# probcomp/PClean

Measured on AMD Instinct MI355X. Metric: rows/sec per Gibbs sweep on 1M-row synthetic hospital; F1 vs ground truth, higher is better.
Workload: dtype f64

## Files before the change

pclean_amd/csrc/sweep.hip:

```cpp
#include "sweep_internal.h"

int g_pclean_sync_count = 0;

__global__ void publish_count_kernel(const unsigned int* __restrict__ src, volatile unsigned int* __restrict__ dst, unsigned int seq) {
  dst[0] = *src;
  __threadfence_system();
  dst[1] = seq;
}
int read_count(pclean_ctx* ctx, const void* dev, void* out, const char* func, int line) {
  SweepState* s = st(ctx);
  static const bool no_poll = getenv("PCLEAN_NO_POLL") != nullptr;
  static const bool trace = getenv("PCLEAN_TRACE_SYNC") != nullptr;
  if (trace) fprintf(stderr, "[pclean sync %d] %s:%d (count)\n", ++g_pclean_sync_count, func, line);
  if (!no_poll && !s->h_poll) {
    if (hipHostMalloc((void**)&s->h_poll, 64, hipHostMallocMapped | hipHostMallocCoherent) != hipSuccess) s->h_poll = nullptr;
    if (s->h_poll) {
      s->h_poll[0] = s->h_poll[1] = 0;
      if (hipHostGetDevicePointer((void**)&s->d_poll, (void*)s->h_poll, 0) != hipSuccess) {
        (void)hipHostFree((void*)s->h_poll);
        s->h_poll = nullptr;
      }
    }
  }
  if (no_poll || !s->h_poll) {
    HIPCHK(ctx, hipMemcpyAsync(out, dev, 4, hipMemcpyDeviceToHost, ctx->stream));
    HIPCHK(ctx, hipStreamSynchronize(ctx->stream));
    return PCLEAN_OK;
  }
  const unsigned int seq = ++s->poll_seq;
  hipLaunchKernelGGL(publish_count_kernel, dim3(1), dim3(1), 0, ctx->stream, (const unsigned int*)dev, s->d_poll, seq);
  if (s->on_first_wait) {
    std::function<int()> f;
    f.swap(s->on_first_wait);
    const int rcf = f();
    if (rcf) return rcf;
  }
  volatile unsigned int* h = s->h_poll;
  for (long spins = 0; h[1] != seq; ++spins)
    if (spins > 2000000) {
      HIPCHK(ctx, hipStreamSynchronize(ctx->stream));
      if (h[1] != seq) return pclean_fail(ctx, PCLEAN_ERR_HIP, "count read-back: the publishing kernel did not run");
    }
  *(unsigned int*)out = h[0];
  return PCLEAN_OK;
}

__device__ int32_t resolve_new_value(const PlanDev& pl, int node, int col, const int32_t* vals) {
  for (int depth = 0; depth < 16; ++depth) {
    const int cn = pl.colmap[2 * (pl.colmap_begin[node] + col)];
    const int cc = pl.colmap[2 * (pl.colmap_begin[node] + col) + 1];
    if (cn < 0) return -1;
    const int choice = vals[cn];
    if (pl.kind[cn] == PCLEAN_NODE_LEAF) return pl.cols[cn][choice];
    if (choice >= 0) return pl.cols[cn][(size_t)cc * pl.n_rows[cn] + choice];
    node = cn;
    col = cc;
  }
  return -1;
}




struct CtxSrc {
  int32_t n_ctx;
  const int32_t* pchoice[PCLEAN_MAX_CTX];
  const int32_t* pnewpos[PCLEAN_MAX_CTX];
  const int32_t* vals[PCLEAN_MAX_CTX];
  int32_t n_nodes[PCLEAN_MAX_CTX];
  const int32_t* root_col[PCLEAN_MAX_CTX];
  int32_t col[PCLEAN_MAX_CTX];
  PlanDev plan[PCLEAN_MAX_CTX];
};

__global__ void gather_ctx_kernel(size_t NP, CtxSrc cs, int32_t* it_ctx) {
  size_t t = (size_t)blockIdx.x * blockDim.x + threadIdx.x;
  if (t >= NP) return;
  for (int s = 0; s < cs.n_ctx; ++s) {
    int32_t v;
    const int choice = cs.pchoice[s][t];
    if (choice >= 0)
      v = cs.root_col[s][choice];
    else
      v = resolve_new_value(cs.plan[s], 0, cs.col[s], cs.vals[s] + (size_t)cs.pnewpos[s][t] * cs.n_nodes[s]);
    it_ctx[(size_t)s * NP + t] = v;
  }
}

__global__ void ctx_count_kernel(int N, int P, int n_ctx, const int32_t* __restrict__ it_ctx, int32_t* __restrict__ rep,
                                 int32_t* __restrict__ n_distinct) {
  const int i = blockIdx.x * blockDim.x + threadIdx.x;
  if (i >= N) return;
  const size_t NP = (size_t)N * P;
  int nd = 0;
  for (int p = 0; p < P; ++p) {
    const size_t sp = (size_t)p * N + i;
    int c[PCLEAN_MAX_CTX];
    for (int k = 0; k < PCLEAN_MAX_CTX; ++k) c[k] = k < n_ctx ? it_ctx[(size_t)k * NP + sp] : 0;
    int q = 0;
    for (; q < p; ++q) {
      bool same = true;
      for (int k = 0; k < PCLEAN_MAX_CTX; ++k)
        if (k < n_ctx) same &= it_ctx[(size_t)k * NP + (size_t)q * N + i] == c[k];
      if (same) break;
    }
    rep[sp] = q;
    nd += q == p ? 1 : 0;
  }
  n_distinct[i] = nd;
}
__global__ void ctx_fill_kernel(int N, int P, int n_ctx, const int32_t* __restrict__ it_ctx, const int32_t* __restrict__ rep,
                                const int32_t* __restrict__ off, const int32_t* __restrict__ cur_b,
                                int32_t* __restrict__ slot_item, int32_t* __restrict__ row, int32_t* __restrict__ ctxv,
                                int32_t* __restrict__ excl) {
  const int i = blockIdx.x * blockDim.x + threadIdx.x;
  if (i >= N) return;
  const size_t NP = (size_t)N * P;
  int j = off[i];
  for (int p = 0; p < P; ++p) {
    const size_t sp = (size_t)p * N + i;
    const int q = rep[sp];
    if (q == p) {
      row[j] = i;
      excl[j] = cur_b ? cur_b[i] : -1;
      for (int k = 0; k < PCLEAN_MAX_CTX; ++k) ctxv[(size_t)j * PCLEAN_MAX_CTX + k] = k < n_ctx ? it_ctx[(size_t)k * NP + sp] : 0;
      slot_item[sp] = j++;
    } else {
      slot_item[sp] = slot_item[(size_t)q * N + i];
    }
  }
}
#define CI_PC 8
__global__ __launch_bounds__(256) void ctx_items_kernel(int N, int P, CtxSrc cs, const int32_t* __restrict__ cur_b,
                                                        int32_t* __restrict__ it_ctx, int32_t* __restrict__ slot_item,
                                                        int32_t* __restrict__ row, int32_t* __restrict__ ctxv,
                                                        int32_t* __restrict__ excl, unsigned int* __restrict__ n_extra,
                                                        int extra_cap) {
  __shared__ unsigned int wcnt[4];
  __shared__ unsigned int bbase;
  const int i = blockIdx.x * blockDim.x + threadIdx.x;
  const int lane = threadIdx.x & 63, wave = threadIdx.x >> 6;
  const size_t NP = (size_t)N * P;
  int c0[PCLEAN_MAX_CTX] = {0, 0, 0, 0};
  static_assert(PCLEAN_MAX_CTX == 4, "c0 initialiser");
  unsigned int mine = 0;
  if (i < N) {
    bool all_same = true;
    for (int p0 = 0; p0 < P; p0 += CI_PC) {
#pragma unroll
      for (int s = 0; s < PCLEAN_MAX_CTX; ++s) {
        if (s >= cs.n_ctx) break;
        int ch[CI_PC];
        int32_t v[CI_PC];
// ... 341 lines not shown
  if (i >= n_rows) return;
  if (only_rows && !only_rows[i]) return;
  FixW<PMAX> f;
  fix_weights<PMAX>(logw + (size_t)i * sr, sp, P, f);
  const uint32_t rr = (uint32_t)((int64_t)i + row_offset);
  const bool csmc = csmc_flag ? (csmc_flag[i] >= 0) : (is_csmc != 0);
  int c;
  if (use_mh && csmc && P >= 2) {
    const double Ud = (double)f.U;
    const double w0 = (double)f.u[0] / Ud, w1 = (double)f.u[PMAX > 1 ? 1 : 0] / Ud;
    double ratio = w1 / (1e-10 + w0);
    if (ratio > 1.0) ratio = 1.0;
    const double x = pclean_u01(pclean_rand64(seed, rr, PCLEAN_SITE_MH, 0u, sweep));
    c = (f.U != 0 && x < ratio) ? 1 : 0;
  } else {
    c = fix_pick<PMAX>(f, P, pclean_rand64(seed, rr, PCLEAN_SITE_FINAL, 0u, sweep));
  }
  chosen[i] = c;
  const double lt = pclean_lse_from_fix(f.m, f.U);
  if (log_total) log_total[i] = lt;
  if (logml) logml[i] = (logml_acc ? logml_acc[i] : 0.0) + lt - pclean_log((double)P);
}


template <int PMAX>
__global__ __launch_bounds__(256) void particle_update_final_kernel(
    int N, int P, const int32_t* __restrict__ draws_rm, const double* __restrict__ lse, const int32_t* __restrict__ slot_item,
    const int32_t* __restrict__ draws_item, const double* __restrict__ lse_item, const int32_t* __restrict__ cur_b,
    int32_t* __restrict__ pchoice, const double* __restrict__ w, int first, int use_mh, const int32_t* __restrict__ csmc_flag,
    uint64_t seed, uint32_t sweep, int64_t row_offset, int32_t* __restrict__ chosen, const double* __restrict__ logml_acc,
    double* __restrict__ logml, const int32_t* __restrict__ skip_rows, int lazy, const double* __restrict__ w_uni) {
  const int i = blockIdx.x * blockDim.x + threadIdx.x;
  if (i >= N) return;
  if (skip_rows && skip_rows[i]) return;
  const int keep = cur_b ? cur_b[i] : -1;
  if (lazy && keep >= 0) pchoice[i] = keep;
  FixW<PMAX> f;
  double wv[PMAX];
  f.m = -__builtin_inf();
  int dv[PMAX];
  double lv[PMAX], wp[PMAX];
  const size_t Ns = (size_t)N;
  if (slot_item) {
    int itm[PMAX];
#pragma unroll
    for (int p = 0; p < PMAX; ++p) itm[p] = slot_item[(size_t)(p < P ? p : P - 1) * Ns + i];
#pragma unroll
    for (int p = 0; p < PMAX; ++p) lv[p] = lse_item[itm[p]];
    if (!lazy) {
#pragma unroll
      for (int p = 0; p < PMAX; ++p) dv[p] = draws_item[(size_t)itm[p] * P + (p < P ? p : P - 1)];
    }
  } else {
    const double l0 = lse[i];
#pragma unroll
    for (int p = 0; p < PMAX; ++p) lv[p] = l0;
    if (!lazy) {
#pragma unroll
      for (int p = 0; p < PMAX; ++p) dv[p] = draws_rm[(size_t)i * P + (p < P ? p : P - 1)];
    }
  }
  if (lazy) {
#pragma unroll
    for (int p = 0; p < PMAX; ++p) dv[p] = 0;
  }
  if (first) {
#pragma unroll
    for (int p = 0; p < PMAX; ++p) wp[p] = 0.0;
  } else if (w_uni) {
    const double wu = 0.0 + w_uni[i];
#pragma unroll
    for (int p = 0; p < PMAX; ++p) wp[p] = wu;
  } else {
#pragma unroll
    for (int p = 0; p < PMAX; ++p) wp[p] = w[(size_t)(p < P ? p : P - 1) * Ns + i];
  }
#pragma unroll
  for (int p = 0; p < PMAX; ++p) {
    wv[p] = 0.0;
    if (p < P) {
      if (!lazy) pchoice[(size_t)p * Ns + i] = (p == 0 && keep >= 0) ? keep : dv[p];
      wv[p] = wp[p] + lv[p];
      f.m = fmax(f.m, wv[p]);
    }
  }
  f.U = 0;
#pragma unroll
  for (int p = 0; p < PMAX; ++p) {
    f.u[p] = (p < P && f.m != -__builtin_inf()) ? pclean_fixw(wv[p] - f.m) : 0ull;
    f.U += f.u[p];
  }
  const uint32_t rr = (uint32_t)((int64_t)i + row_offset);
  const bool csmc = csmc_flag[i] >= 0;
  int c;
  if (use_mh && csmc && P >= 2) {
    const double Ud = (double)f.U;
    const double w0 = (double)f.u[0] / Ud, w1 = (double)f.u[PMAX > 1 ? 1 : 0] / Ud;
    double ratio = w1 / (1e-10 + w0);
    if (ratio > 1.0) ratio = 1.0;
    const double x = pclean_u01(pclean_rand64(seed, rr, PCLEAN_SITE_MH, 0u, sweep));
    c = (f.U != 0 && x < ratio) ? 1 : 0;
  } else {
    c = fix_pick<PMAX>(f, P, pclean_rand64(seed, rr, PCLEAN_SITE_FINAL, 0u, sweep));
  }
  chosen[i] = c;
  logml[i] = logml_acc[i] + pclean_lse_from_fix(f.m, f.U) - pclean_log((double)P);
}

__global__ __launch_bounds__(256) void finalize_block_kernel(int n_rows, const int32_t* chosen, const int32_t* pchoice,
                                                             const int32_t* pnewpos, const int32_t* cur_b,
                                                             int32_t* choice, int32_t* chosen_newpos,
                                                             unsigned long long* stats, int hist_rows,
                                                             int32_t* moved_flag, int32_t* new_flag,
                                                             unsigned int* __restrict__ wg_moved,
                                                             unsigned int* __restrict__ wg_new) {
  extern __shared__ int32_t hist[];
  for (int k = threadIdx.x; k < hist_rows; k += 256) hist[k] = 0;
  if (hist_rows) __syncthreads();
  int i = blockIdx.x * blockDim.x + threadIdx.x;
  int is_moved = 0, is_new = 0;
  if (i < n_rows) {
    const size_t s = (size_t)chosen[i] * n_rows + i;
    const int c = pchoice[s];
    const int o = cur_b[i];
    choice[i] = c;
    const int np = c == PCLEAN_CHOICE_NEW ? pnewpos[s] : -1;
    chosen_newpos[i] = np;
    new_flag[i] = is_new = np >= 0 ? 1 : 0;
    moved_flag[i] = is_moved = c != o ? 1 : 0;
    if (o != c) {
      if (hist_rows) {
        if (o >= 0) atomicAdd(&hist[o], -1);
        if (c >= 0) atomicAdd(&hist[c], 1);
      } else {
        if (o >= 0) atomicAdd(&stats[o], (unsigned long long)(-1ll));
        if (c >= 0) atomicAdd(&stats[c], 1ull);
      }
    }
  }
  if (hist_rows) {
    __syncthreads();
    for (int k = threadIdx.x; k < hist_rows; k += 256) {
      const int v = hist[k];
      if (v) atomicAdd(&stats[k], (unsigned long long)(long long)v);
    }
  }
  const int n_moved = __syncthreads_count(is_moved), n_newr = __syncthreads_count(is_new);
  if (threadIdx.x == 0) {
    wg_moved[blockIdx.x] = (unsigned int)n_moved;
    wg_new[blockIdx.x] = (unsigned int)n_newr;
  }
}

#define TAIL_MAX_LISTS (2 * PCLEAN_MAX_BLOCKS)
__global__ __launch_bounds__(1024) void tail_scan_kernel(int nb, unsigned int* __restrict__ wg_cnt, int32_t* __restrict__ totals) {
  __shared__ unsigned int wsum[16];
  unsigned int* c = wg_cnt + (size_t)blockIdx.x * nb;
  const int lane = threadIdx.x & 63, wave = threadIdx.x >> 6;
  unsigned int carry = 0;
  for (int base = 0; base < nb; base += 1024) {
    const int j = base + threadIdx.x;
    const unsigned int v = j < nb ? c[j] : 0u;
    unsigned int incl = v;
    for (int o = 1; o < 64; o <<= 1) {
      const unsigned int x = __shfl_up(incl, o, 64);
      if (lane >= o) incl += x;
    }
    if (lane == 63) wsum[wave] = incl;
    __syncthreads();
    unsigned int wbase = 0, tot = 0;
    for (int k = 0; k < 16; ++k) {
      if (k < wave) wbase += wsum[k];
      tot += wsum[k];
    }
    if (j < nb) c[j] = carry + wbase + incl - v;
    carry += tot;
    __syncthreads();
  }
  if (threadIdx.x == 0) totals[blockIdx.x] = (int32_t)carry;
}
struct TailLists {
  const int32_t* flag[TAIL_MAX_LISTS];
  int32_t* list[TAIL_MAX_LISTS];
};
__global__ __launch_bounds__(256) void tail_scatter_kernel(int n_rows, int nb, TailLists tl, const unsigned int* __restrict__ wg_off) {
  __shared__ unsigned int wcnt[4];
  const int l = blockIdx.y;
  const int32_t* flag = tl.flag[l];
  if (!flag) return;
  const int i = blockIdx.x * 256 + threadIdx.x;
  const int lane = threadIdx.x & 63, wave = threadIdx.x >> 6;
  const bool f = i < n_rows && flag[i] != 0;
  const unsigned long long mk = __ballot(f);
  if (lane == 0) wcnt[wave] = (unsigned int)__popcll(mk);
  __syncthreads();
  if (!f) return;
  unsigned int pos = wg_off[(size_t)l * nb + blockIdx.x] + (unsigned int)__popcll(mk & ((1ull << lane) - 1ull));
  for (int w = 0; w < wave; ++w) pos += wcnt[w];
  tl.list[l][pos] = i;
}

__global__ void gauss_prior_kernel(int n_rows, int P, GaussDev g0, const GaussDev* __restrict__ more, int n_more, PlanDev plan,
                                   const int32_t* __restrict__ pchoice,
                                   const int32_t* __restrict__ pnewpos, const int32_t* __restrict__ vals, int n_nodes,
                                   const int32_t* __restrict__ cur_b, const int32_t* __restrict__ cur_locals, uint64_t seed,
                                   uint32_t sweep, uint32_t block, int64_t row_offset, double* __restrict__ w,
                                   int32_t* __restrict__ plocals) {
  const size_t slot = (size_t)blockIdx.x * blockDim.x + threadIdx.x;
  if (slot >= (size_t)n_rows * P) return;
  const int p = (int)(slot / (size_t)n_rows), i = (int)(slot % (size_t)n_rows);
  const int choice = pchoice[slot];
  const int32_t* v = choice >= 0 ? nullptr : vals + (size_t)pnewpos[slot] * n_nodes;
  const bool keep = p == 0 && cur_b && cur_b[i] >= 0 && cur_locals;
  const uint32_t rr = (uint32_t)((int64_t)i + row_offset);
  int l[2] = {0, 0}, out[2] = {-1, -1};
  double s = 0.0;
  for (int k = 0; k < g0.n_locals; ++k) {
    const int o = g0.local_obs[k] ? g0.local_obs[k][i] : -1;
    if (o >= 0) {
      l[k] = o;
      s += g0.local_logp[k];
    } else if (keep && cur_locals[2 * (size_t)i + k] >= 0) {
      l[k] = cur_locals[2 * (size_t)i + k];
    } else {
      l[k] = (int)pclean_mulhi64(pclean_rand64(seed, rr, PCLEAN_SITE_LOCALS(block), (uint32_t)p | ((uint32_t)(k + 1) << 16), sweep),
                                 (uint64_t)g0.local_n[k]);
    }
    out[k] = l[k];
  }
  plocals[2 * slot] = out[0];
  plocals[2 * slot + 1] = out[1];
  for (int t = 0; t <= n_more; ++t) {
    const GaussDev& g = t == 0 ? g0 : more[t - 1];
    const double xv = g.x[i];
    if (xv == xv) {
      int idx = 0;
      for (int d = 0; d < g.n_dims; ++d) {
        int val;
        if (g.src_kind[d] == PCLEAN_GSRC_LOCAL)
          val = l[g.src_slot[d]];
        else if (g.src_kind[d] == PCLEAN_GSRC_CAND)
          val = choice >= 0 ? g.src_ptr[d][choice] : resolve_new_value(plan, 0, g.src_slot[d], v);
        else
          val = g.src_ptr[d][i];
        idx += g.stride[d] * val;
      }
      const int u = g.t_kind == PCLEAN_GSRC_LOCAL ? l[g.t_src] : 0;
      s += gauss_normal_logpdf(g.tx[u] ? g.tx[u][i] : xv * g.t_scale[u], g.mu[idx], g.sigma, g.log_sigma);
      s -= g.tl[u] ? g.tl[u][i] : g.t_lad[u];
    }
  }
  w[slot] += s;
}
__global__ void locals_pick_kernel(int n_rows, const int32_t* __restrict__ chosen, const int32_t* __restrict__ plocals,
                                   int32_t* __restrict__ locals) {
  const int i = blockIdx.x * blockDim.x + threadIdx.x;
  if (i >= n_rows) return;
  const size_t slot = (size_t)chosen[i] * n_rows + i;
  locals[2 * i] = plocals[2 * slot];
  locals[2 * i + 1] = plocals[2 * slot + 1];
}

__global__ void locals_tail_kernel(int n_rows, int P, GaussDev g, const GaussDev* __restrict__ more, int n_more, PlanDev plan,
                                   const int32_t* chosen,
                                   const int32_t* pchoice, const int32_t* pnewpos, const int32_t* vals, int n_nodes,
                                   uint64_t seed, uint32_t sweep, uint32_t block, int64_t row_offset, int32_t* locals) {
  int i = blockIdx.x * blockDim.x + threadIdx.x;
  if (i >= n_rows) return;
  const int c = chosen[i];
  const size_t slot = (size_t)c * n_rows + i;
  const int choice = pchoice[slot];
  const int32_t* v = choice >= 0 ? nullptr : vals + (size_t)pnewpos[slot] * n_nodes;
  locals[2 * i] = locals[2 * i + 1] = -1;
  double sc[16];
  int codes[16];
  int n = gauss_combo_scores(
      g, more, n_more, i, nullptr,
      [&](const GaussDev& gt, int d) -> int {
        if (gt.src_kind[d] == PCLEAN_GSRC_CAND)
          return choice >= 0 ? gt.src_ptr[d][choice] : resolve_new_value(plan, 0, gt.src_slot[d], v);
        return gt.src_ptr[d][i];
      },
      sc, codes);
  if (n == 0) {
    for (int l0 = 0; l0 < g.local_n[0]; ++l0)
      for (int l1 = 0; l1 < g.local_n[1]; ++l1) {
        const bool ok0 = !g.local_obs[0] || g.local_obs[0][i] < 0 || g.local_obs[0][i] == l0;
        const bool ok1 = !g.local_obs[1] || g.local_obs[1][i] < 0 || g.local_obs[1][i] == l1;
        if (ok0 && ok1) {
          sc[n] = 0.0;
          codes[n] = l0 * 16 + l1;
          ++n;
        }
      }
  }
  double m = -__builtin_inf();
  for (int k = 0; k < n; ++k) m = fmax(m, sc[k]);
  uint64_t u[16], U = 0;
  for (int k = 0; k < n; ++k) {
    u[k] = m == -__builtin_inf() ? 0ull : pclean_fixw(sc[k] - m);
    U += u[k];
  }
  int pick = n - 1;
  if (U) {
    const uint64_t x = pclean_mulhi64(
        pclean_rand64(seed, (uint32_t)((int64_t)i + row_offset), PCLEAN_SITE_LOCALS(block), (uint32_t)c, sweep), U);
    uint64_t acc = 0;
// ... 1131 lines not shown
      if (!rep || !n_distinct || !off || !tmp) return pclean_fail(ctx, PCLEAN_ERR_HIP, "scratch alloc failed");
      {
        ProfScope ps(ctx, "ctx_items");
        hipLaunchKernelGGL(gather_ctx_kernel, grid1(NP), dim3(256), 0, ctx->stream, NP, cs, r.it_ctx.p);
        HIPCHK(ctx, hipMemsetAsync(n_distinct + N, 0, sizeof(int32_t), ctx->stream));
        hipLaunchKernelGGL(ctx_count_kernel, grid1(N), dim3(256), 0, ctx->stream, N, P, (int)b.n_ctx, r.it_ctx.p, rep, n_distinct);
        HIPCHK(ctx, hipcub::DeviceScan::ExclusiveSum(tmp, tmp_scan, n_distinct, off, N + 1, ctx->stream));
        PCLEAN_READ_COUNT(ctx, off + N, &n_items);
      }
      d_row = scratch<int32_t>(ctx, n_items);
      d_ctx = scratch<int32_t>(ctx, (size_t)n_items * PCLEAN_MAX_CTX);
      d_excl = scratch<int32_t>(ctx, n_items);
      if (!d_row || !d_ctx || !d_excl) return pclean_fail(ctx, PCLEAN_ERR_HIP, "scratch alloc failed");
      hipLaunchKernelGGL(ctx_fill_kernel, grid1(N), dim3(256), 0, ctx->stream, N, P, (int)b.n_ctx, r.it_ctx.p, rep, off, cur_b, slot_item,
                         d_row, d_ctx, d_excl);
      }
      double* lse_item = scratch<double>(ctx, n_items);
      int32_t* draws_item = scratch<int32_t>(ctx, (size_t)n_items * P);
      if (!lse_item || !draws_item) return pclean_fail(ctx, PCLEAN_ERR_HIP, "scratch alloc failed");
      il = ItemList{(int)n_items, d_row, d_ctx, nullptr, nullptr};
      if (!no_fused_items) il.n_primary = N;
      if (fuse_final || split_final) s->lazy_req = SweepState::LazyReq{true, split_final ? emit_rows : nullptr};
      rc = eval_node(ctx, bi, 0, il, d_excl, seed, sweep_idx, P, lse_item, draws_item, nullptr, nullptr, bi == ctx->timed_block);
      s->lazy_req = SweepState::LazyReq();
      if (rc) return rc;
      if (bi == ctx->timed_block) {
        hot_timed = true;
        ctx->timing.hot_kernel_launches += 1;
      }
      lazy = s->lazy_out;
      s->lazy_out.valid = false;
      lazy.args.slot_item = slot_item;
      ProfScope ps(ctx, "particle_update");
      if (fuse_final) {
        DISPATCH_PMAX(P, hipLaunchKernelGGL(particle_update_final_kernel<PMAX>, grid1(N), dim3(256), 0, ctx->stream, N, P,
                                            (const int32_t*)nullptr, (const double*)nullptr, slot_item, draws_item, lse_item, cur_b,
                                            r.pchoice.p, s->w.p, (w_by_first_block && bi == 0) ? 1 : 0, use_mh, cur_base, seed,
                                            sweep_idx, s->row_offset + ctx->active_begin, s->chosen.p, s->logml_acc.p, s->logml.p,
                                            (const int32_t*)nullptr, lazy.valid ? 1 : 0, w_uni));
        final_fused = true;
        { const int rcl = lazy_draws(); if (rcl) return rcl; }
      } else {
      n_new_ctr = fresh_counter(ctx);
      if (!n_new_ctr) return pclean_fail(ctx, PCLEAN_ERR_HIP, "counter bank: device alloc failed");
      hipLaunchKernelGGL(particle_update_kernel, dim3((N + PU_T - 1) / PU_T), dim3(PU_T), 0, ctx->stream, N, P, (const int32_t*)nullptr,
                         (const double*)nullptr, slot_item, draws_item, lse_item, cur_b, r.pchoice.p, s->w.p,
                         n_new_ctr, r.new_slots.p, r.pnewpos.p, (w_by_first_block && bi == 0) ? 1 : 0, emit_rows, split_final ? 1 : 0, 0,
                         w_uni, 0);
      if (!split_final) w_uni = nullptr;
      if (split_final) {
        DISPATCH_PMAX(P, hipLaunchKernelGGL(particle_update_final_kernel<PMAX>, grid1(N), dim3(256), 0, ctx->stream, N, P,
                                            (const int32_t*)nullptr, (const double*)nullptr, slot_item, draws_item, lse_item, cur_b,
                                            r.pchoice.p, s->w.p, (w_by_first_block && bi == 0) ? 1 : 0, use_mh, cur_base, seed,
                                            sweep_idx, s->row_offset + ctx->active_begin, s->chosen.p, s->logml_acc.p, s->logml.p,
                                            emit_rows, lazy.valid ? 1 : 0, w_uni));
        final_only_rows = emit_rows;
        { const int rcl = lazy_draws(); if (rcl) return rcl; }
      }
      }
    }
    if (!prefetch_started) {
      const int rcp = start_prefetch();
      if (rcp) return rcp;
    }
    unsigned int n_new = 0;
    if (!final_fused) PCLEAN_READ_COUNT(ctx, n_new_ctr, &n_new);
    const bool degenerate_rows = (n_new & 0x80000000u) != 0u;
    n_new &= 0x7fffffffu;
    r.n_new = final_fused ? -1 : (int)n_new;
    r.lazy_new = final_fused || (bi == n_blocks - 1 && !eager_all && (!drawable || emit_rows != nullptr));
    if (r.lazy_new && !emit_rows) n_new = 0;
    if (emit_rows) r.n_new = -1;
    if (r.vals.alloc(std::max<size_t>((size_t)n_new * nn, 1))) return pclean_fail(ctx, PCLEAN_ERR_HIP, "device alloc failed");
    if (n_new) {
      ProfScope ps(ctx, "new_row_sampling");
      const int32_t* list = r.new_slots.p;
      hipLaunchKernelGGL(fill_i32_kernel, grid1((size_t)n_new * nn), dim3(256), 0, ctx->stream, r.vals.p,
                         (size_t)n_new * nn, -2);
      int32_t* row = scratch<int32_t>(ctx, n_new);
      int32_t* cx = scratch<int32_t>(ctx, (size_t)n_new * PCLEAN_MAX_CTX);
      int32_t* part = scratch<int32_t>(ctx, n_new);
      int32_t* org = scratch<int32_t>(ctx, n_new);
      int32_t* ex = scratch<int32_t>(ctx, n_new);
      if (!row || !cx || !part || !org || !ex) return pclean_fail(ctx, PCLEAN_ERR_HIP, "scratch alloc failed");
      hipLaunchKernelGGL(rootlist_items_kernel, grid1(n_new), dim3(256), 0, ctx->stream, (int)n_new, N, NP, list,
                         has_ctx ? r.it_ctx.p : nullptr, cur_b, row, cx, part, org, ex);
      hipLaunchKernelGGL(set_col_kernel, grid1(n_new), dim3(256), 0, ctx->stream, (int)n_new, nn, 0,
                         (int32_t)PCLEAN_CHOICE_NEW, r.vals.p);
      ItemList sub{(int)n_new, row, cx, part, org};
      rc = sample_children(ctx, bi, 0, sub, ex, seed, sweep_idx, r.vals.p, nn);
      if (rc) return rc;
      if (prior_mode) {
        ctx->prior_mode = false;
        const NodeDev* nds;
        const int32_t *dnc, *dcb, *dch;
        rc = upload_plan_nodes(ctx, bi, &nds, &dnc, &dcb, &dch);
        if (!rc)
          rc = pclean_launch_prior_terms(ctx, NP, N, nn, nds, dnc, dcb, dch, r.pchoice.p, r.pnewpos.p, r.vals.p,
                                         has_ctx ? r.it_ctx.p : nullptr, s->w.p);
        if (!rc) rc = gauss_prior();
        if (rc) return rc;
      }
      if (drawable) {
        if (!split_final) materialise_w();
        rc = apply_dummy_corrections(ctx, bi, r.new_slots.p, r.vals.p, (int)n_new, N, seed, sweep_idx, s->w.p);
        if (rc) return rc;
      }
    } else if (prior_mode) {
      ctx->prior_mode = false;
      const NodeDev* nds;
      const int32_t *dnc, *dcb, *dch;
      rc = upload_plan_nodes(ctx, bi, &nds, &dnc, &dcb, &dch);
      if (!rc)
        rc = pclean_launch_prior_terms(ctx, NP, N, nn, nds, dnc, dcb, dch, r.pchoice.p, r.pnewpos.p, r.vals.p,
                                       has_ctx ? r.it_ctx.p : nullptr, s->w.p);
      if (!rc) rc = gauss_prior();
      if (rc) return rc;
    }
    ctx->prior_mode = false;

    const int grp_here = b.group >= 0 ? b.group : bi;
    const int grp_next = bi + 1 < n_blocks ? (ctx->block[bi + 1].group >= 0 ? ctx->block[bi + 1].group : bi + 1) : -2;
    const bool equal_weights = bi == 0 && w_by_first_block && !has_ctx && !prior_mode && !(drawable && n_new > 0) && !degenerate_rows;
    static const bool always_resample = getenv("PCLEAN_ALWAYS_RESAMPLE") != nullptr;
    if (!use_mh && bi < n_blocks - 1 && grp_here != grp_next && (!equal_weights || always_resample)) {
      ProfScope ps(ctx, "resample");
      materialise_w();
      DISPATCH_PMAX(P, hipLaunchKernelGGL(maybe_resample_kernel<PMAX>, grid1(N), dim3(256), 0, ctx->stream, N, P, s->w.p,
                                          (size_t)1, (size_t)N, 1, cur_b, seed, sweep_idx, (uint32_t)bi,
                                          s->row_offset + ctx->active_begin, s->ancestors.p, s->logml_inc.p,
                                          (double*)nullptr, s->did.p));
      AncestorArrays arrs{};
      int n_arr = 0;
      for (int k = 0; k <= bi; ++k) {
        if (ctx->block[k].is_score) continue;
        arrs.p[n_arr++] = s->run[k].pchoice.p;
        arrs.p[n_arr++] = s->run[k].pnewpos.p;
        if (s->run[k].plocals_on) arrs.pairs[arrs.n_pairs++] = reinterpret_cast<int64_t*>(s->run[k].plocals.p);
      }
      hipLaunchKernelGGL(apply_ancestors_kernel, grid1(N), dim3(256), 0, ctx->stream, N, P, s->ancestors.p, n_arr, arrs, s->w.p,
                         s->did.p, s->logml_inc.p, s->logml_acc.p);
    }
  }

  if (prefetching) HIPCHK(ctx, hipStreamWaitEvent(ctx->stream, s->pre_join, 0));
  {
    ProfScope ps(ctx, "final_choice_and_outputs");
    if (!final_fused && !final_only_rows) materialise_w();
    if (!final_fused)
    DISPATCH_PMAX(P, hipLaunchKernelGGL(final_choice_kernel<PMAX>, grid1(N), dim3(256), 0, ctx->stream, N, P, s->w.p,
                                        (size_t)1, (size_t)N, use_mh, 1, cur_base, seed, sweep_idx,
                                        s->row_offset + ctx->active_begin, s->chosen.p, (double*)nullptr,
                                        s->logml_acc.p, s->logml.p, final_only_rows));
    for (int bi = 0; bi < n_blocks; ++bi) {
      BlockRun& r = s->run[bi];
      Block& bb = ctx->block[bi];
      if (bb.is_score || !r.lazy_new || r.n_new == 0) continue;
      ProfScope ps2(ctx, "new_row_sampling_chosen");
      const int nn = (int)bb.nodes.size();
      const int32_t* cur_b = cur_base + (size_t)bi * cur_ld;
      unsigned int* cnt_ctr = fresh_counter(ctx);
      hipLaunchKernelGGL(chosen_new_kernel, grid1(N), dim3(256), 0, ctx->stream, N, s->chosen.p, r.pchoice.p, cnt_ctr,
                         r.new_slots.p, r.pnewpos.p);
      unsigned int cnt = 0;
      PCLEAN_READ_COUNT(ctx, cnt_ctr, &cnt);
      if (r.vals.alloc(std::max<size_t>((size_t)cnt * nn, 1))) return pclean_fail(ctx, PCLEAN_ERR_HIP, "device alloc failed");
      if (!cnt) continue;
      hipLaunchKernelGGL(fill_i32_kernel, grid1((size_t)cnt * nn), dim3(256), 0, ctx->stream, r.vals.p, (size_t)cnt * nn, -2);
      int32_t* row = scratch<int32_t>(ctx, cnt);
      int32_t* cx = scratch<int32_t>(ctx, (size_t)cnt * PCLEAN_MAX_CTX);
      int32_t* part = scratch<int32_t>(ctx, cnt);
      int32_t* org = scratch<int32_t>(ctx, cnt);
      int32_t* ex = scratch<int32_t>(ctx, cnt);
      if (!row || !cx || !part || !org || !ex) return pclean_fail(ctx, PCLEAN_ERR_HIP, "scratch alloc failed");
      hipLaunchKernelGGL(rootlist_items_kernel, grid1(cnt), dim3(256), 0, ctx->stream, (int)cnt, N, NP, r.new_slots.p,
                         bb.n_ctx > 0 ? r.it_ctx.p : nullptr, cur_b, row, cx, part, org, ex);
      hipLaunchKernelGGL(set_col_kernel, grid1(cnt), dim3(256), 0, ctx->stream, (int)cnt, nn, 0, (int32_t)PCLEAN_CHOICE_NEW,
                         r.vals.p);
      ItemList sub{(int)cnt, row, cx, part, org};
      int rc = sample_children(ctx, bi, 0, sub, ex, seed, sweep_idx, r.vals.p, nn);
      if (rc) return rc;
    }
    const int nb_wg = (N + 255) / 256;
    unsigned int* wg_cnt = scratch<unsigned int>(ctx, (size_t)2 * n_blocks * nb_wg);
    if (!wg_cnt) return pclean_fail(ctx, PCLEAN_ERR_HIP, "scratch alloc failed");
    TailLists tl{};
    {
      ZeroList zl{};
      for (int bi = 0; bi < n_blocks; ++bi) {
        if (ctx->block[bi].is_score) continue;
        CandTable& rt = ctx->cand[ctx->block[bi].nodes[0].table];
        bool seen = false;
        for (int k = 0; k < zl.n; ++k) seen |= zl.p[k] == (void*)rt.stats.p;
        if (!seen) zero_list_add(ctx, zl, rt.stats.p, (size_t)std::max(rt.n_rows, 1) * 8);
      }
      const int rcz = zero_list_flush(ctx, zl);
      if (rcz) return rcz;
    }
    for (int bi = 0; bi < n_blocks; ++bi) {
      BlockRun& r = s->run[bi];
      Block& bb = ctx->block[bi];
      bb.locals_host.clear();
      r.locals_rows = 0;
      if (bb.is_score) continue;
      const int32_t* cur_b = cur_base + (size_t)bi * cur_ld;
      CandTable& rt = ctx->cand[bb.nodes[0].table];
      const int rows_in_use = (rt.n_used > 0 && rt.n_used <= rt.n_rows) ? std::min(rt.n_rows, (rt.n_used + 63) & ~63) : rt.n_rows;
      static const bool no_hist = getenv("PCLEAN_NO_HIST") != nullptr;
      const int hist_rows = (rt.n_rows <= 12288 && !no_hist) ? rows_in_use : 0;
      hipLaunchKernelGGL(finalize_block_kernel, grid1(N), dim3(256), (size_t)hist_rows * sizeof(int32_t), ctx->stream, N,
                         s->chosen.p, r.pchoice.p, r.pnewpos.p, cur_b, r.choice.p, r.chosen_newpos.p,
                         (unsigned long long*)rt.stats.p, hist_rows, r.moved_flag.p, r.new_flag.p,
                         wg_cnt + (size_t)(2 * bi) * nb_wg, wg_cnt + (size_t)(2 * bi + 1) * nb_wg);
      tl.flag[2 * bi] = r.moved_flag.p;
      tl.list[2 * bi] = r.moved_list.p;
      tl.flag[2 * bi + 1] = r.new_flag.p;
      tl.list[2 * bi + 1] = r.new_list.p;
      if (choice)
        HIPCHK(ctx, hipMemcpyAsync(choice + (size_t)bi * N, r.choice.p, (size_t)N * 4, hipMemcpyDeviceToHost, ctx->stream));
      if (!bb.node_gauss.empty() && bb.node_gauss[0] >= 0 && bb.gauss[bb.node_gauss[0]].n_locals > 0) {
        if (r.locals.alloc((size_t)N * 2)) return pclean_fail(ctx, PCLEAN_ERR_HIP, "device alloc failed");
        if (r.plocals_on) {
          hipLaunchKernelGGL(locals_pick_kernel, grid1(N), dim3(256), 0, ctx->stream, N, s->chosen.p, r.plocals.p, r.locals.p);
        } else {
          GaussDev gd;
          const GaussDev* gmore;
          int n_gmore;
          int rc = build_gauss_dev(ctx, bb.gauss[bb.node_gauss[0]], &rt, gd);
          if (!rc) rc = build_gauss_more(ctx, bb, 0, &rt, &gmore, &n_gmore);
          if (rc) return rc;
          hipLaunchKernelGGL(locals_tail_kernel, grid1(N), dim3(256), 0, ctx->stream, N, P, gd, gmore, n_gmore, r.plan, s->chosen.p,
                             r.pchoice.p, r.pnewpos.p, r.vals.p, (int)bb.nodes.size(), seed, sweep_idx, (uint32_t)bi,
                             s->row_offset + ctx->active_begin, r.locals.p);
        }
        r.locals_rows = N;
        if (!defer) {
          bb.locals_host.resize((size_t)N * 2);
          HIPCHK(ctx, hipMemcpyAsync(bb.locals_host.data(), r.locals.p, (size_t)N * 8, hipMemcpyDeviceToHost, ctx->stream));
        }
      }
    }
    {
      for (int bi = 0; bi < n_blocks; ++bi)
        if (ctx->block[bi].is_score)
          HIPCHK(ctx, hipMemsetAsync(wg_cnt + (size_t)(2 * bi) * nb_wg, 0, (size_t)2 * nb_wg * sizeof(unsigned int), ctx->stream));
      hipLaunchKernelGGL(tail_scan_kernel, dim3(2 * n_blocks), dim3(1024), 0, ctx->stream, nb_wg, wg_cnt, s->tail_counts.p);
      hipLaunchKernelGGL(tail_scatter_kernel, dim3(nb_wg, 2 * n_blocks), dim3(256), 0, ctx->stream, N, nb_wg, tl, wg_cnt);
    }
    (void)hipEventRecord(s->eve, ctx->stream);
    if (chosen_particle) HIPCHK(ctx, hipMemcpyAsync(chosen_particle, s->chosen.p, (size_t)N * 4, hipMemcpyDeviceToHost, ctx->stream));
    if (logml) HIPCHK(ctx, hipMemcpyAsync(logml, s->logml.p, (size_t)N * 8, hipMemcpyDeviceToHost, ctx->stream));
  }
  s->last_hot_timed = hot_timed;
  s->outputs_pending = true;
  s->lists_on_host = false;
  {
    const Block& b0 = ctx->block[(ctx->timed_block >= 0 && ctx->timed_block < n_blocks && !ctx->block[ctx->timed_block].is_score) ? ctx->timed_block : 0];
    const double F = b0.nodes[0].n_terms, K = ctx->cand[b0.nodes[0].table].n_rows;
    ctx->timing.hot_kernel_alg_bytes = (double)N * (4.0 * F + (K + 1.0) * (8.0 * F + 4.0) + 8.0 * P);
  }
  if (defer) return PCLEAN_OK;
  int rcf = pclean_sweep_finish_queue(ctx);
  if (rcf) return rcf;
  PCLEAN_SYNC(ctx);
  rcf = pclean_sweep_finish_synced(ctx);
  if (rcf) return rcf;
  if (choice)
    for (int bi = 0; bi < n_blocks; ++bi)
      if (ctx->block[bi].is_score)
        for (int i = 0; i < N; ++i) choice[(size_t)bi * N + i] = 0;
  return pclean_sweep_fetch_lists(ctx);
}

int pclean_sweep_finish_queue(pclean_ctx* ctx) {
  SweepState* s = st(ctx);
  if (!s->outputs_pending) return PCLEAN_OK;
  int rc = d2h_small(ctx, s->h_counts, s->tail_counts.p, 2 * s->last_blocks * sizeof(int32_t));
  if (rc) return rc;
  const int rco = queue_over_copy(ctx);
  if (rco) return rco;
  s->h_counts[3 * PCLEAN_MAX_BLOCKS] = 0;
  if (s->dummy_used) rc = d2h_small(ctx, s->h_counts + 3 * PCLEAN_MAX_BLOCKS, s->dummy_ctr.p + 1, sizeof(int32_t), s->h_counts);
  if (rc) return rc;
  return d2h_flush(ctx);
}
int pclean_sweep_finish_synced(pclean_ctx* ctx) {
  SweepState* s = st(ctx);
  if (!s->outputs_pending) return PCLEAN_OK;
  s->outputs_pending = false;
  apply_over_stats(ctx);
  if (s->prof_on) prof_collect(ctx);
  float tot = 0;
  HIPCHK(ctx, hipEventElapsedTime(&tot, s->evs, s->eve));
  ctx->timing.total_ms = tot;
  ctx->timing.hot_kernel_ms = 0.f;
  if (s->last_hot_timed) {
    float ms = 0;
    HIPCHK(ctx, hipEventElapsedTime(&ms, s->ev0, s->ev1));
    ctx->timing.hot_kernel_ms = ms;
    if (s->gate_timed) {
      float mg = 0;
      HIPCHK(ctx, hipEventElapsedTime(&mg, s->evg0, s->evg1));
      ctx->timing.hot_kernel_ms += mg;
    }
  }
  if (s->h_counts[3 * PCLEAN_MAX_BLOCKS])
    return pclean_fail(ctx, PCLEAN_ERR_CAPACITY, "pclean_sweep: an observed string longer than %d symbols below a chosen "
                                                 "dummy value", DUMMY_MAX_LEN);
  return PCLEAN_OK;
}
int pclean_sweep_fetch_lists(pclean_ctx* ctx) {
  SweepState* s = st(ctx);
  if (s->lists_on_host) return PCLEAN_OK;
  for (int bi = 0; bi < s->last_blocks; ++bi) {
    BlockRun& r = s->run[bi];
    Block& b = ctx->block[bi];
    const int nn = (int)b.nodes.size();
    b.new_rows_host.clear();
    b.new_vals_host.clear();
    b.moved_rows_host.clear();
    b.moved_choice_host.clear();
    if (b.is_score) continue;
    const int n_moved = s->h_counts[2 * bi], n_newrows = s->h_counts[2 * bi + 1];
    if (n_moved > 0) {
      int32_t* ch_d = scratch<int32_t>(ctx, n_moved);
      if (!ch_d) return pclean_fail(ctx, PCLEAN_ERR_HIP, "scratch alloc failed");
      hipLaunchKernelGGL(gather_moved_kernel, grid1(n_moved), dim3(256), 0, ctx->stream, n_moved, r.moved_list.p,
                         r.choice.p, ch_d);
      b.moved_rows_host.resize(n_moved);
      b.moved_choice_host.resize(n_moved);
      HIPCHK(ctx, hipMemcpyAsync(b.moved_rows_host.data(), r.moved_list.p, (size_t)n_moved * 4, hipMemcpyDeviceToHost, ctx->stream));
      HIPCHK(ctx, hipMemcpyAsync(b.moved_choice_host.data(), ch_d, (size_t)n_moved * 4, hipMemcpyDeviceToHost, ctx->stream));
    }
    if (n_newrows > 0) {
      int32_t* rows_d = scratch<int32_t>(ctx, n_newrows);
      int32_t* vals_d = scratch<int32_t>(ctx, (size_t)n_newrows * nn);
      if (!rows_d || !vals_d) return pclean_fail(ctx, PCLEAN_ERR_HIP, "scratch alloc failed");
      hipLaunchKernelGGL(gather_new_rows_kernel, grid1(n_newrows), dim3(256), 0, ctx->stream, n_newrows, r.new_list.p,
                         r.chosen_newpos.p, r.vals.p, nn, s->chosen.p, rows_d, vals_d);
      b.new_rows_host.resize(n_newrows);
      b.new_vals_host.resize((size_t)n_newrows * nn);
      HIPCHK(ctx, hipMemcpyAsync(b.new_rows_host.data(), rows_d, (size_t)n_newrows * 4, hipMemcpyDeviceToHost, ctx->stream));
      HIPCHK(ctx, hipMemcpyAsync(b.new_vals_host.data(), vals_d, (size_t)n_newrows * nn * 4, hipMemcpyDeviceToHost, ctx->stream));
    }
  }
  PCLEAN_SYNC(ctx);
  s->lists_on_host = true;
  return PCLEAN_OK;
}

extern "C" int pclean_sweep_fetch(pclean_ctx* ctx) {
  if (!ctx) return PCLEAN_ERR_ARG;
  HIPCHK(ctx, hipSetDevice(ctx->device));
  int rc = pclean_sweep_finish_queue(ctx);
  if (rc) return rc;
  PCLEAN_SYNC(ctx);
  rc = pclean_sweep_finish_synced(ctx);
  if (rc) return rc;
  return pclean_sweep_fetch_lists(ctx);
}

extern "C" int pclean_set_sweep_mode(pclean_ctx* ctx, int32_t flags) {
  if (!ctx || flags < 0 || flags > 1) return pclean_fail(ctx, PCLEAN_ERR_ARG, "pclean_set_sweep_mode: bad flags");
  ctx->defer_outputs = (flags & 1) != 0;
  return PCLEAN_OK;
}

extern "C" int pclean_get_new_rows(pclean_ctx* ctx, int32_t block_id, int32_t* n_out, int32_t* rows_out,
                                   int32_t* vals_out) {
  if (!ctx || block_id < 0 || block_id >= PCLEAN_MAX_BLOCKS || !ctx->block[block_id].valid || !n_out)
    return pclean_fail(ctx, PCLEAN_ERR_ARG, "pclean_get_new_rows: bad arguments");
  const Block& b = ctx->block[block_id];
  *n_out = (int32_t)b.new_rows_host.size();
  if (rows_out && !b.new_rows_host.empty()) memcpy(rows_out, b.new_rows_host.data(), b.new_rows_host.size() * 4);
  if (vals_out && !b.new_vals_host.empty()) memcpy(vals_out, b.new_vals_host.data(), b.new_vals_host.size() * 4);
  return PCLEAN_OK;
}

extern "C" int pclean_get_moved(pclean_ctx* ctx, int32_t block_id, int32_t* n_out, int32_t* rows_out,
                                int32_t* choice_out) {
  if (!ctx || block_id < 0 || block_id >= PCLEAN_MAX_BLOCKS || !ctx->block[block_id].valid || !n_out)
    return pclean_fail(ctx, PCLEAN_ERR_ARG, "pclean_get_moved: bad arguments");
  const Block& b = ctx->block[block_id];
  *n_out = (int32_t)b.moved_rows_host.size();
  if (rows_out && !b.moved_rows_host.empty()) memcpy(rows_out, b.moved_rows_host.data(), b.moved_rows_host.size() * 4);
  if (choice_out && !b.moved_choice_host.empty())
    memcpy(choice_out, b.moved_choice_host.data(), b.moved_choice_host.size() * 4);
  return PCLEAN_OK;
}

extern "C" int pclean_set_cur_locals(pclean_ctx* ctx, int32_t block_id, const int32_t* locals, int32_t n_rows) {
  if (!ctx || block_id < 0 || block_id >= PCLEAN_MAX_BLOCKS || !ctx->block[block_id].valid)
    return pclean_fail(ctx, PCLEAN_ERR_ARG, "pclean_set_cur_locals: bad arguments");
  Block& b = ctx->block[block_id];
  if (!locals || n_rows <= 0) {
    b.cur_locals.release();
    b.cur_locals_rows = 0;
    return PCLEAN_OK;
  }
  if (n_rows != ctx->n_rows) return pclean_fail(ctx, PCLEAN_ERR_ARG, "pclean_set_cur_locals: one pair per observed row (%d), got %d", ctx->n_rows, n_rows);
// ... 174 lines not shown
```

Before: 445.2 million.

## Fuse per-block finalize and chosen-NEW listing into one persistent tail kernel

Replaces the per-block finalize_block_kernel launches and the separate chosen_new_kernel plus blocking count read with one persistent 2D-grid kernel. The kernel walks 256-row tiles per workgroup, lists chosen NEW rows using wave-aggregated atomics, and keeps one shared histogram per workgroup instead of one per 256-row block. Sampling of chosen new rows is deferred until after the tail scan and scatter, so the host sync on the count no longer sits between finalize launches. This cuts launches, host round trips and global histogram atomics, at the cost of fewer workgroups (about half the CU count) and a changed, nondeterministic slot order for new rows.

```diff
diff --git a/pclean_amd/csrc/sweep.hip b/pclean_amd/csrc/sweep.hip
--- a/pclean_amd/csrc/sweep.hip
+++ b/pclean_amd/csrc/sweep.hip
@@ -1,4 +1,5 @@
 #include "sweep_internal.h"
+#include "tail_tiles.h"
 
 int g_pclean_sync_count = 0;
 
@@ -646,7 +647,123 @@
   }
 }
 
+struct TailBlock {
+  const int32_t* pchoice;
+  int32_t* pnewpos;
+  const int32_t* cur_b;
+  int32_t* choice;
+  int32_t* chosen_newpos;
+  unsigned long long* stats;
+  int32_t* moved_flag;
+  int32_t* new_flag;
+  unsigned int* wg_moved;
+  unsigned int* wg_new;
+  unsigned int* new_ctr;
+  int32_t* new_slots;
+  int32_t hist_rows, on, lazy, pad;
+};
+struct TailBlocks {
+  TailBlock b[PCLEAN_MAX_BLOCKS];
+};
+#define TAIL_WG_THREADS 1024
+#define TAIL_STEP (TAIL_WG_THREADS / TAIL_TILE_ROWS)
+__global__ __launch_bounds__(TAIL_WG_THREADS) void finalize_tail_kernel(int n_rows, int n_tiles, const int32_t* __restrict__ chosen,
+                                                                        TailBlocks tb) {
+  extern __shared__ int32_t hist[];
+  __shared__ unsigned int wcnt[2][2][TAIL_WG_THREADS / 64];
+  const TailBlock& b = tb.b[blockIdx.y];
+  if (!b.on) return;
+  const TailTileRange tr = tail_tile_range(n_tiles, (int)gridDim.x, (int)blockIdx.x);
+  if (tr.begin >= tr.end) return;
+  const int hist_rows = b.hist_rows;
+  const int lane = threadIdx.x & 63, wave = threadIdx.x >> 6;
+  const int sub = threadIdx.x / TAIL_TILE_ROWS, in_tile = threadIdx.x % TAIL_TILE_ROWS;
+  for (int k = threadIdx.x; k < hist_rows; k += TAIL_WG_THREADS) hist[k] = 0;
+  if (hist_rows) __syncthreads();
+  int ch_next = 0, o_next = 0;
+  {
+    const int i0 = (tr.begin + sub) * TAIL_TILE_ROWS + in_tile;
+    if (tr.begin + sub < tr.end && i0 < n_rows) {
+      ch_next = chosen[i0];
+      o_next = b.cur_b[i0];
+    }
+  }
+  for (int t0 = tr.begin; t0 < tr.end; t0 += TAIL_STEP) {
+    const int tile = t0 + sub;
+    const bool mine = tile < tr.end;
+    const int i = mine ? tile * TAIL_TILE_ROWS + in_tile : n_rows;
+    const int par = ((t0 - tr.begin) / TAIL_STEP) & 1;
+    bool is_moved = false, is_new = false, wants_pos = false;
+    size_t s = 0;
+    int c = 0;
+    const int ch = ch_next, o = o_next;
+    {
+      const int i1 = (tile + TAIL_STEP) * TAIL_TILE_ROWS + in_tile;
+      if (tile + TAIL_STEP < tr.end && i1 < n_rows) {
+        ch_next = chosen[i1];
+        o_next = b.cur_b[i1];
+      }
+    }
+    if (i < n_rows) {
+      s = (size_t)ch * n_rows + i;
+      c = b.pchoice[s];
+      wants_pos = b.lazy && c == PCLEAN_CHOICE_NEW;
+    }
+    int np = -1;
+    if (b.lazy) {
+      const unsigned long long mk = __ballot(wants_pos);
+      if (mk) {
+        unsigned int base = 0;
+        if (lane == __builtin_ctzll(mk)) base = atomicAdd(b.new_ctr, (unsigned int)__popcll(mk));
+        base = __shfl(base, __builtin_ctzll(mk), 64);
+        if (wants_pos) {
+          np = (int)(base + (unsigned int)__popcll(mk & ((1ull << lane) - 1ull)));
+          b.new_slots[np] = (int32_t)s;
+          b.pnewpos[s] = np;
+        }
+      }
+    } else if (i < n_rows && c == PCLEAN_CHOICE_NEW) {
+      np = b.pnewpos[s];
+    }
+    if (i < n_rows) {
+      b.choice[i] = c;
+      b.chosen_newpos[i] = np;
+      is_new = np >= 0;
+      is_moved = c != o;
+      b.new_flag[i] = is_new ? 1 : 0;
+      b.moved_flag[i] = is_moved ? 1 : 0;
+      if (o != c) {
+        if (hist_rows) {
+          if (o >= 0) atomicAdd(&hist[o], -1);
+          if (c >= 0) atomicAdd(&hist[c], 1);
+        } else {
+          if (o >= 0) atomicAdd(&b.stats[o], (unsigned long long)(-1ll));
+          if (c >= 0) atomicAdd(&b.stats[c], 1ull);
+        }
+      }
+    }
+    const unsigned long long mm = __ballot(is_moved), mn = __ballot(is_new);
+    if (lane == 0) {
+      wcnt[par][0][wave] = (unsigned int)__popcll(mm);
+      wcnt[par][1][wave] = (unsigned int)__popcll(mn);
+    }
+    __syncthreads();
+    if (in_tile == 0 && mine) {
+      b.wg_moved[tile] = wcnt[par][0][wave] + wcnt[par][0][wave + 1] + wcnt[par][0][wave + 2] + wcnt[par][0][wave + 3];
+      b.wg_new[tile] = wcnt[par][1][wave] + wcnt[par][1][wave + 1] + wcnt[par][1][wave + 2] + wcnt[par][1][wave + 3];
+    }
+  }
+  if (hist_rows) {
+    __syncthreads();
+    for (int k = threadIdx.x; k < hist_rows; k += TAIL_WG_THREADS) {
+      const int v = hist[k];
+      if (v) atomicAdd(&b.stats[k], (unsigned long long)(long long)v);
+    }
+  }
+}
+
 #define TAIL_MAX_LISTS (2 * PCLEAN_MAX_BLOCKS)
+#define TAIL_CUS_PER_WG 2
 __global__ __launch_bounds__(1024) void tail_scan_kernel(int nb, unsigned int* __restrict__ wg_cnt, int32_t* __restrict__ totals) {
   __shared__ unsigned int wsum[16];
   unsigned int* c = wg_cnt + (size_t)blockIdx.x * nb;
@@ -2084,20 +2201,22 @@
                                         (size_t)1, (size_t)N, use_mh, 1, cur_base, seed, sweep_idx,
                                         s->row_offset + ctx->active_begin, s->chosen.p, (double*)nullptr,
                                         s->logml_acc.p, s->logml.p, final_only_rows));
-    for (int bi = 0; bi < n_blocks; ++bi) {
+    static const bool no_fused_finalize = getenv("PCLEAN_NO_FUSED_FINALIZE") != nullptr;
+    static const int forced_tail_wgs = getenv("PCLEAN_TAIL_WGS") ? std::max(1, atoi(getenv("PCLEAN_TAIL_WGS"))) : 0;
+    static const bool trace_tail = getenv("PCLEAN_TRACE_SYNC") != nullptr;
+    unsigned int* chosen_ctr[PCLEAN_MAX_BLOCKS] = {};
+    auto sample_chosen = [&](int bi) -> int {
       BlockRun& r = s->run[bi];
       Block& bb = ctx->block[bi];
-      if (bb.is_score || !r.lazy_new || r.n_new == 0) continue;
       ProfScope ps2(ctx, "new_row_sampling_chosen");
       const int nn = (int)bb.nodes.size();
       const int32_t* cur_b = cur_base + (size_t)bi * cur_ld;
-      unsigned int* cnt_ctr = fresh_counter(ctx);
-      hipLaunchKernelGGL(chosen_new_kernel, grid1(N), dim3(256), 0, ctx->stream, N, s->chosen.p, r.pchoice.p, cnt_ctr,
-                         r.new_slots.p, r.pnewpos.p);
       unsigned int cnt = 0;
-      PCLEAN_READ_COUNT(ctx, cnt_ctr, &cnt);
+      PCLEAN_READ_COUNT(ctx, chosen_ctr[bi], &cnt);
+      if (trace_tail) fprintf(stderr, "[pclean tail] block %d: %u chosen NEW rows listed by %s\n", bi, cnt,
+                              no_fused_finalize ? "chosen_new_kernel" : "finalize_tail_kernel");
       if (r.vals.alloc(std::max<size_t>((size_t)cnt * nn, 1))) return pclean_fail(ctx, PCLEAN_ERR_HIP, "device alloc failed");
-      if (!cnt) continue;
+      if (!cnt) return PCLEAN_OK;
       hipLaunchKernelGGL(fill_i32_kernel, grid1((size_t)cnt * nn), dim3(256), 0, ctx->stream, r.vals.p, (size_t)cnt * nn, -2);
       int32_t* row = scratch<int32_t>(ctx, cnt);
       int32_t* cx = scratch<int32_t>(ctx, (size_t)cnt * PCLEAN_MAX_CTX);
@@ -2110,10 +2229,20 @@
       hipLaunchKernelGGL(set_col_kernel, grid1(cnt), dim3(256), 0, ctx->stream, (int)cnt, nn, 0, (int32_t)PCLEAN_CHOICE_NEW,
                          r.vals.p);
       ItemList sub{(int)cnt, row, cx, part, org};
-      int rc = sample_children(ctx, bi, 0, sub, ex, seed, sweep_idx, r.vals.p, nn);
+      return sample_children(ctx, bi, 0, sub, ex, seed, sweep_idx, r.vals.p, nn);
+    };
+    for (int bi = 0; bi < n_blocks; ++bi) {
+      BlockRun& r = s->run[bi];
+      if (ctx->block[bi].is_score || !r.lazy_new || r.n_new == 0) continue;
+      chosen_ctr[bi] = fresh_counter(ctx);
+      if (!chosen_ctr[bi]) return pclean_fail(ctx, PCLEAN_ERR_HIP, "counter bank: device alloc failed");
+      if (!no_fused_finalize) continue;
+      hipLaunchKernelGGL(chosen_new_kernel, grid1(N), dim3(256), 0, ctx->stream, N, s->chosen.p, r.pchoice.p, chosen_ctr[bi],
+                         r.new_slots.p, r.pnewpos.p);
+      const int rc = sample_chosen(bi);
       if (rc) return rc;
     }
-    const int nb_wg = (N + 255) / 256;
+    const int nb_wg = (N + TAIL_TILE_ROWS - 1) / TAIL_TILE_ROWS;
     unsigned int* wg_cnt = scratch<unsigned int>(ctx, (size_t)2 * n_blocks * nb_wg);
     if (!wg_cnt) return pclean_fail(ctx, PCLEAN_ERR_HIP, "scratch alloc failed");
     TailLists tl{};
@@ -2129,6 +2258,8 @@
       const int rcz = zero_list_flush(ctx, zl);
       if (rcz) return rcz;
     }
+    TailBlocks tb{};
+    int max_hist = 0;
     for (int bi = 0; bi < n_blocks; ++bi) {
       BlockRun& r = s->run[bi];
       Block& bb = ctx->block[bi];
@@ -2140,14 +2271,70 @@
       const int rows_in_use = (rt.n_used > 0 && rt.n_used <= rt.n_rows) ? std::min(rt.n_rows, (rt.n_used + 63) & ~63) : rt.n_rows;
       static const bool no_hist = getenv("PCLEAN_NO_HIST") != nullptr;
       const int hist_rows = (rt.n_rows <= 12288 && !no_hist) ? rows_in_use : 0;
-      hipLaunchKernelGGL(finalize_block_kernel, grid1(N), dim3(256), (size_t)hist_rows * sizeof(int32_t), ctx->stream, N,
-                         s->chosen.p, r.pchoice.p, r.pnewpos.p, cur_b, r.choice.p, r.chosen_newpos.p,
-                         (unsigned long long*)rt.stats.p, hist_rows, r.moved_flag.p, r.new_flag.p,
-                         wg_cnt + (size_t)(2 * bi) * nb_wg, wg_cnt + (size_t)(2 * bi + 1) * nb_wg);
+      if (no_fused_finalize) {
+        hipLaunchKernelGGL(finalize_block_kernel, grid1(N), dim3(256), (size_t)hist_rows * sizeof(int32_t), ctx->stream, N,
+                           s->chosen.p, r.pchoice.p, r.pnewpos.p, cur_b, r.choice.p, r.chosen_newpos.p,
+                           (unsigned long long*)rt.stats.p, hist_rows, r.moved_flag.p, r.new_flag.p,
+                           wg_cnt + (size_t)(2 * bi) * nb_wg, wg_cnt + (size_t)(2 * bi + 1) * nb_wg);
+      } else {
+        TailBlock& t = tb.b[bi];
+        t.pchoice = r.pchoice.p;
+        t.pnewpos = r.pnewpos.p;
+        t.cur_b = cur_b;
+        t.choice = r.choice.p;
+        t.chosen_newpos = r.chosen_newpos.p;
+        t.stats = (unsigned long long*)rt.stats.p;
+        t.moved_flag = r.moved_flag.p;
+        t.new_flag = r.new_flag.p;
+        t.wg_moved = wg_cnt + (size_t)(2 * bi) * nb_wg;
+        t.wg_new = wg_cnt + (size_t)(2 * bi + 1) * nb_wg;
+        t.new_ctr = chosen_ctr[bi];
+        t.new_slots = r.new_slots.p;
+        t.hist_rows = hist_rows;
+        t.on = 1;
+        t.lazy = chosen_ctr[bi] ? 1 : 0;
+        max_hist = std::max(max_hist, hist_rows);
+      }
       tl.flag[2 * bi] = r.moved_flag.p;
       tl.list[2 * bi] = r.moved_list.p;
       tl.flag[2 * bi + 1] = r.new_flag.p;
       tl.list[2 * bi + 1] = r.new_list.p;
+    }
+    if (!no_fused_finalize) {
+      static int tail_cap = 0;
+      if (!tail_cap) {
+        int n_cu = 256;
+        hipDeviceProp_t prop;
+        if (hipGetDeviceProperties(&prop, ctx->device) == hipSuccess && prop.multiProcessorCount > 0) n_cu = prop.multiProcessorCount;
+        tail_cap = std::max(1, n_cu / TAIL_CUS_PER_WG);
+      }
+      const int n_wgs = tail_wg_count(nb_wg, tail_cap, forced_tail_wgs);
+      if (trace_tail)
+        fprintf(stderr, "[pclean tail] finalize_tail_kernel: %d tiles, %d workgroups per block, at most %d tiles per workgroup\n",
+                nb_wg, n_wgs, (nb_wg + n_wgs - 1) / n_wgs);
+      hipLaunchKernelGGL(finalize_tail_kernel, dim3(n_wgs, n_blocks), dim3(TAIL_WG_THREADS), (size_t)max_hist * sizeof(int32_t), ctx->stream, N,
+                         nb_wg, s->chosen.p, tb);
+    } else if (trace_tail) {
+      fprintf(stderr, "[pclean tail] finalize_block_kernel: one launch per block\n");
+    }
+    {
+      for (int bi = 0; bi < n_blocks; ++bi)
+        if (ctx->block[bi].is_score)
+          HIPCHK(ctx, hipMemsetAsync(wg_cnt + (size_t)(2 * bi) * nb_wg, 0, (size_t)2 * nb_wg * sizeof(unsigned int), ctx->stream));
+      hipLaunchKernelGGL(tail_scan_kernel, dim3(2 * n_blocks), dim3(1024), 0, ctx->stream, nb_wg, wg_cnt, s->tail_counts.p);
+      hipLaunchKernelGGL(tail_scatter_kernel, dim3(nb_wg, 2 * n_blocks), dim3(256), 0, ctx->stream, N, nb_wg, tl, wg_cnt);
+    }
+    if (!no_fused_finalize)
+      for (int bi = 0; bi < n_blocks; ++bi)
+        if (chosen_ctr[bi]) {
+          const int rc = sample_chosen(bi);
+          if (rc) return rc;
+        }
+    for (int bi = 0; bi < n_blocks; ++bi) {
+      BlockRun& r = s->run[bi];
+      Block& bb = ctx->block[bi];
+      if (bb.is_score) continue;
+      CandTable& rt = ctx->cand[bb.nodes[0].table];
       if (choice)
         HIPCHK(ctx, hipMemcpyAsync(choice + (size_t)bi * N, r.choice.p, (size_t)N * 4, hipMemcpyDeviceToHost, ctx->stream));
       if (!bb.node_gauss.empty() && bb.node_gauss[0] >= 0 && bb.gauss[bb.node_gauss[0]].n_locals > 0) {
@@ -2171,13 +2358,6 @@
           HIPCHK(ctx, hipMemcpyAsync(bb.locals_host.data(), r.locals.p, (size_t)N * 8, hipMemcpyDeviceToHost, ctx->stream));
         }
       }
-    }
-    {
-      for (int bi = 0; bi < n_blocks; ++bi)
-        if (ctx->block[bi].is_score)
-          HIPCHK(ctx, hipMemsetAsync(wg_cnt + (size_t)(2 * bi) * nb_wg, 0, (size_t)2 * nb_wg * sizeof(unsigned int), ctx->stream));
-      hipLaunchKernelGGL(tail_scan_kernel, dim3(2 * n_blocks), dim3(1024), 0, ctx->stream, nb_wg, wg_cnt, s->tail_counts.p);
-      hipLaunchKernelGGL(tail_scatter_kernel, dim3(nb_wg, 2 * n_blocks), dim3(256), 0, ctx->stream, N, nb_wg, tl, wg_cnt);
     }
     (void)hipEventRecord(s->eve, ctx->stream);
     if (chosen_particle) HIPCHK(ctx, hipMemcpyAsync(chosen_particle, s->chosen.p, (size_t)N * 4, hipMemcpyDeviceToHost, ctx->stream));
diff --git a/pclean_amd/csrc/tail_tiles.h b/pclean_amd/csrc/tail_tiles.h
--- /dev/null
+++ b/pclean_amd/csrc/tail_tiles.h
@@ -0,0 +1,26 @@
+#pragma once
+
+#define TAIL_TILE_ROWS 256
+
+struct TailTileRange {
+  int begin, end;
+};
+
+#if defined(__HIPCC__)
+__host__ __device__
+#endif
+static inline TailTileRange tail_tile_range(int n_tiles, int n_wgs, int wg) {
+  TailTileRange r{0, 0};
+  if (n_tiles <= 0 || n_wgs <= 0 || wg < 0 || wg >= n_wgs) return r;
+  const int base = n_tiles / n_wgs, rem = n_tiles % n_wgs;
+  r.begin = wg * base + (wg < rem ? wg : rem);
+  r.end = r.begin + base + (wg < rem ? 1 : 0);
+  return r;
+}
+
+static inline int tail_wg_count(int n_tiles, int cap, int forced) {
+  if (n_tiles <= 0) return 1;
+  int n = forced > 0 ? forced : cap;
+  if (n < 1) n = 1;
+  return n < n_tiles ? n : n_tiles;
+}
```

After: 460.5 million (median of 6 runs). 3.4% higher.
